# hyrise/hyrise

Measured on AMD Instinct MI355X. Metric: rows/sec TableScan+JoinHash, TPC-H SF10 lineitem, higher is better.
Workload: dtype u16

## Files before the change

hyrise_amd/csrc/join.hip:

```cpp
#include "hy_device.hpp"
#include "hy_decode.hpp"
#include "hy_arithmetic.hpp"
#include "hy_scan_job.hpp"

#include <algorithm>
#include <atomic>
#include <cmath>
#include <chrono>
#include <cstring>
#include <type_traits>

namespace hy {

constexpr uint32_t JOIN_TILE = 4096;
constexpr uint32_t JOIN_THREADS = 512;
constexpr uint32_t JOIN_WAVES = JOIN_THREADS / 64;
constexpr uint32_t JOIN_WAVE_ROWS = JOIN_TILE / JOIN_WAVES;
constexpr uint32_t JOIN_ROUNDS = JOIN_WAVE_ROWS / 64;
constexpr uint32_t JOIN_STAGE = JOIN_TILE + 256;
constexpr uint32_t MAX_PARTITIONS = 256;
typedef uint32_t u32x2_t __attribute__((ext_vector_type(2)));
typedef uint32_t u32x4_t __attribute__((ext_vector_type(4)));
constexpr uint32_t PROBE_SIZE_PER_CHUNK = 65535u * 2u;
constexpr uint32_t BLOOM_BITS = 1u << 20;
// ... 2140 lines not shown
  hipLaunchKernelGGL(scan_blocks, dim3(n_blocks), dim3(256), 0, stream, in, n, sums.as<uint64_t>(), out);
  return HY_OK;
}


struct JoinMailbox {
  uint64_t key_or, first_key, last_key;
  uint64_t key_min, key_max;
  uint32_t unsorted, any_null, equal_neighbours, duplicate;
  uint32_t unsorted_signed, build_unconfirmed;
  uint64_t n_pairs;
  uint32_t n_slices, n_uncached, fits;
  uint32_t error;
};
static thread_local JoinMailbox* t_mailbox = nullptr;
static thread_local JoinMailbox* t_mailbox_dev = nullptr;

struct BuildVerdict {
  uint64_t key_min, key_max;
  uint32_t unsorted_signed, equal_neighbours, outside_hint, done;
};

struct ZeroedBlocks {
  void* table = nullptr;
  size_t table_capacity = 0;
  void* filter = nullptr;
  size_t dirty_table = 0, dirty_filter = 0;
  bool clean = false;
  hipStream_t stream = nullptr;
};
static thread_local ZeroedBlocks t_zeroed[2];

static void free_zeroed_blocks() {
  for (ZeroedBlocks& z : t_zeroed) {
    if (z.table) (void)hipFree(z.table);
    if (z.filter) (void)hipFree(z.filter);
    z = ZeroedBlocks{};
  }
}

void release_thread_join_state() {
  if (t_mailbox) (void)hipHostFree(t_mailbox);
  t_mailbox = t_mailbox_dev = nullptr;
  free_zeroed_blocks();
}

static hy_status join_mailbox(JoinMailbox** host, JoinMailbox** device) {
  if (!t_mailbox) {
    static_assert(sizeof(JoinMailbox) <= 256, "the mailbox is a 256-byte pinned block");
    HY_HIP(hipHostMalloc(reinterpret_cast<void**>(&t_mailbox), 256, hipHostMallocMapped));
    HY_HIP(hipHostGetDevicePointer(reinterpret_cast<void**>(&t_mailbox_dev), t_mailbox, 0));
  }
  std::memset(t_mailbox, 0, sizeof(JoinMailbox));
  *host = t_mailbox;
  *device = t_mailbox_dev;
  return HY_OK;
}

// ... 216 lines not shown
    low = other_low < low ? other_low : low;
    high = other_high > high ? other_high : high;
  }
  __syncthreads();
  if ((tid & 63) == 0) { s_min[tid >> 6] = low; s_max[tid >> 6] = high; atomicOr(&s_flags, static_cast<uint32_t>(bits)); }
  __syncthreads();
  if (tid != 0) return;
  for (uint32_t w = 0; w < 4; ++w) { low = s_min[w] < low ? s_min[w] : low; high = s_max[w] > high ? s_max[w] : high; }
  verdict->key_min = low ^ SIGN;
  verdict->key_max = high ^ SIGN;
  verdict->unsorted_signed = s_flags & 1u ? 1 : 0;
  verdict->equal_neighbours = s_flags & 2u ? 1 : 0;
  verdict->outside_hint = s_flags & 4u ? 1 : 0;
  verdict->done = 1;
  __threadfence_system();
}

constexpr uint32_t FW_STEP = 512;
constexpr uint32_t FW_STEPS_PER_SLICE = SLICE_ROWS / FW_STEP;
constexpr uint32_t FW_WINDOW = 2048;
static_assert(HY_FOR_BLOCK_SIZE % FW_STEP == 0, "a step lies in one FrameOfReference block");

constexpr uint32_t FW_BATCH = 4;

struct FillWaveState {
  uint64_t unsorted = 0, equal = 0, outside = 0;
  int32_t low = 0x7FFFFFFF, high = static_cast<int32_t>(0x80000000u);
  bool any_rows = false;
  int32_t carry = 0;
  bool has_carry = false;
};

template <uint32_t WIDTH>
__device__ __forceinline__ int32_t fill_step_key(const u32x4_t& a, const u32x4_t& b, uint32_t bias, uint32_t j) {
  uint32_t stored;
  if constexpr (WIDTH == 4) stored = j < 4 ? a[j] : b[j - 4];
  else if constexpr (WIDTH == 2) stored = (a[j / 2] >> (16 * (j & 1))) & 0xFFFFu;
  else stored = (a[j / 4] >> (8 * (j & 3))) & 0xFFu;
  return static_cast<int32_t>(stored + bias);
}

__device__ __forceinline__ bool key_in_front_of_step(const MaterializeArgs& a, uint32_t step, int32_t* key) {
  uint32_t slice = step / FW_STEPS_PER_SLICE;
  const uint32_t offset = (step % FW_STEPS_PER_SLICE) * FW_STEP;
  if (offset > 0) {
    const SliceView view = a.views[slice];
    if (view.row_count > 0) { *key = view_key(view, view.row_begin + (offset <= view.row_count ? offset : view.row_count) - 1); return true; }
  }
  while (slice-- > 0) {
    const SliceView earlier = a.views[slice];
    if (earlier.row_count == 0) continue;
    *key = view_key(earlier, earlier.row_begin + earlier.row_count - 1);
    return true;
  }
  return false;
}

__device__ __forceinline__ void fill_flush_window(const uint32_t* bits_window, uint32_t span, uint32_t first_word, uint32_t origin_word, uint32_t first_rank, bool first_is_leader, uint32_t lane,
                                                  u32x2_entry_t* entries, uint32_t* bloom_words, uint32_t debug) {
  uint32_t keys_before = 0;
  for (uint32_t begin = 0; begin < span; begin += 64) {
    const uint32_t i = begin + lane;
    const uint32_t bits = i < span ? bits_window[i] : 0u;
    const uint32_t count = __popc(bits);
    uint32_t inclusive = count;
#pragma unroll
    for (int d = 1; d < 64; d <<= 1) {
      const uint32_t other = __shfl_up(inclusive, d, 64);
      if (lane >= static_cast<uint32_t>(d)) inclusive += other;
    }
    const uint32_t base = first_rank + keys_before + inclusive - count;
    keys_before += __builtin_amdgcn_readlane(inclusive, 63);
    if (i >= span) continue;
    const uint32_t table_word = first_word + i;
    if (bits && bloom_words) atomicOr(bloom_words + ((table_word + origin_word) & (BLOOM_BITS / 32 - 1)), bits);
#ifdef HY_DEBUG_SWITCHES
    if (debug & 2) { if (bits == 0xDEADBEEFu && base == 0x12345678u) entries[0] = u32x2_entry_t{bits, base}; continue; }
#endif
    if (i == 0 || i + 1 == span) {
      if (bits) atomicOr(reinterpret_cast<uint32_t*>(entries + table_word), bits);
      if (bits && (i != 0 || first_is_leader)) reinterpret_cast<uint32_t*>(entries + table_word)[1] = base;
    } else {
      entries[table_word] = u32x2_entry_t{bits, bits ? base : 0u};
    }
  }
}

template <uint32_t WIDTH, uint32_t K>
__device__ __forceinline__ bool fill_process_steps(FillWaveState& w, const u32x4_t (&a)[K], const u32x4_t (&b)[K], const uint32_t (&bias)[K], const uint32_t (&rows)[K],
                                                   const uint32_t (&first_rank)[K], uint32_t lane, uint32_t origin, uint32_t range, u32x2_entry_t* entries, uint32_t* bloom_words,
                                                   uint32_t* bits_window, uint32_t debug) {
  const uint32_t origin_word = origin >> 5;
  if (rows[0] == 0) return true;
  int32_t key[K][8];
  uint32_t lane_rows[K];
  int32_t first_key = 0, last_key = 0;
#pragma unroll
  for (uint32_t k = 0; k < K; ++k) {
#pragma unroll
    for (uint32_t j = 0; j < 8; ++j) key[k][j] = fill_step_key<WIDTH>(a[k], b[k], bias[k], j);
    lane_rows[k] = lane * 8 < rows[k] ? (rows[k] - lane * 8 < 8 ? rows[k] - lane * 8 : 8) : 0;
    if (rows[k] != 0) {
      const uint32_t last_lane = (rows[k] - 1) >> 3, last_j = (rows[k] - 1) & 7;
      int32_t mine = key[k][0];
#pragma unroll
      for (uint32_t j = 1; j < 8; ++j) mine = last_j == j ? key[k][j] : mine;
      last_key = __builtin_amdgcn_readlane(mine, last_lane);
    }
    if (k == 0) first_key = __builtin_amdgcn_readfirstlane(key[0][0]);
  }
  const uint32_t first_rel = static_cast<uint32_t>(first_key) - origin, last_rel = static_cast<uint32_t>(last_key) - origin;
  const uint32_t first_word = first_rel >> 5;
  const bool windowed = first_rel <= range && last_rel <= range && last_rel >= first_rel && (last_rel >> 5) - first_word < FW_WINDOW;
  if (K > 1 && !windowed) return false;
  const uint32_t span = windowed ? (last_rel >> 5) - first_word + 1 : 0;
  if (!w.any_rows) w.low = first_key;
  w.high = last_key;
  w.any_rows = true;
  int32_t before[K];
  bool first_has_before[K];
  {
    int32_t carry = w.carry;
    bool has_carry = w.has_carry;
#pragma unroll
    for (uint32_t k = 0; k < K; ++k) {
      before[k] = __shfl_up(key[k][7], 1, 64);
      if (lane == 0) before[k] = carry;
      first_has_before[k] = lane != 0 || has_carry;
#pragma unroll
      for (uint32_t j = 0; j < 8; ++j) {
        const int32_t previous = j == 0 ? before[k] : key[k][j - 1];
        const bool checked = j < lane_rows[k] && (j != 0 || first_has_before[k]);
        w.unsorted |= __ballot(checked && key[k][j] < previous);
        w.equal |= __ballot(checked && key[k][j] == previous);
      }
      if (rows[k] != 0) {
        carry = __builtin_amdgcn_readlane(key[k][7], 63);
        has_carry = true;
      }
    }
  }
  const uint32_t carry_rel = static_cast<uint32_t>(w.carry) - origin;
  const bool first_is_leader = !w.has_carry || carry_rel > range || (carry_rel >> 5) != first_word;
  w.carry = last_key;
  w.has_carry = true;
  if (first_rel > range || last_rel > range) w.outside = 1;
#ifdef HY_DEBUG_SWITCHES
  if (debug & 8) return true;
#endif
  if (windowed) {
#ifdef HY_DEBUG_SWITCHES
    if (debug & 4) return true;
#endif
    for (uint32_t i = lane; i < span; i += 64) bits_window[i] = 0;
    __builtin_amdgcn_fence(__ATOMIC_RELEASE, "wavefront");
    __builtin_amdgcn_wave_barrier();
#pragma unroll
    for (uint32_t k = 0; k < K; ++k) {
#pragma unroll
      for (uint32_t j = 0; j < 8; ++j) {
        const uint32_t rel = static_cast<uint32_t>(key[k][j]) - origin;
        const uint32_t at = (rel >> 5) - first_word;
        if (j < lane_rows[k] && at < span) atomicOr(&bits_window[at], 1u << (rel & 31));
      }
    }
    __builtin_amdgcn_fence(__ATOMIC_RELEASE, "wavefront");
    __builtin_amdgcn_wave_barrier();
    __builtin_amdgcn_fence(__ATOMIC_ACQUIRE, "wavefront");
    fill_flush_window(bits_window, span, first_word, origin_word, first_rank[0], first_is_leader, lane, entries, bloom_words, debug);
    __builtin_amdgcn_wave_barrier();
  } else {
#pragma unroll
    for (uint32_t k = 0; k < K; ++k) {
      const uint32_t lane_rank = first_rank[k] + lane * 8;
#pragma unroll
      for (uint32_t j = 0; j < 8; ++j) {
        const uint32_t rel = static_cast<uint32_t>(key[k][j]) - origin;
        const int32_t previous = j == 0 ? before[k] : key[k][j - 1];
        const bool has_previous = j != 0 || first_has_before[k];
        w.outside |= __ballot(j < lane_rows[k] && rel > range);
        if (j < lane_rows[k] && rel <= range) {
          const uint32_t table_word = rel >> 5, bits = 1u << (rel & 31);
          atomicOr(reinterpret_cast<uint32_t*>(entries + table_word), bits);
          const uint32_t previous_rel = static_cast<uint32_t>(previous) - origin;
          if (!has_previous || previous_rel > range || (previous_rel >> 5) != table_word) reinterpret_cast<uint32_t*>(entries + table_word)[1] = lane_rank + j;
          if (bloom_words) atomicOr(bloom_words + ((table_word + origin_word) & (BLOOM_BITS / 32 - 1)), bits);
        }
      }
    }
  }
  return true;
}

template <uint32_t WIDTH>
struct FillBatch {
  u32x4_t a[FW_BATCH], b[FW_BATCH];
  uint32_t bias[FW_BATCH], rows[FW_BATCH], first_rank[FW_BATCH];
};

template <uint32_t WIDTH>
__device__ __forceinline__ void load_fill_batch(const MaterializeArgs& a, uint32_t batch_step, uint32_t end_step, uint32_t chunk_rows, uint32_t lane, FillBatch<WIDTH>& batch) {
  typedef const __attribute__((address_space(1))) u32x4_t* global_x4;
  typedef const __attribute__((address_space(1))) u32x2_t* global_x2;
  const uint32_t slice0 = batch_step / FW_STEPS_PER_SLICE;
  const SliceView view0 = a.views[slice0];
  const SliceView view1 = a.views[slice0 + 1 < a.n_slices ? slice0 + 1 : slice0];
  const uint32_t rank0 = view0.chunk * chunk_rows + view0.row_begin, rank1 = view1.chunk * chunk_rows + view1.row_begin;
#pragma unroll
  for (uint32_t k = 0; k < FW_BATCH; ++k) {
    const uint32_t step = batch_step + k;
    const bool second = step / FW_STEPS_PER_SLICE != slice0;
    const SliceView& view = second ? view1 : view0;
    const uint32_t offset = (step % FW_STEPS_PER_SLICE) * FW_STEP;
    batch.rows[k] = step < end_step && view.row_count > offset ? (view.row_count - offset < FW_STEP ? view.row_count - offset : FW_STEP) : 0;
    batch.first_rank[k] = (second ? rank1 : rank0) + offset;
    batch.a[k] = u32x4_t{0, 0, 0, 0};
    batch.b[k] = u32x4_t{0, 0, 0, 0};
    batch.bias[k] = 0;
    if (batch.rows[k] != 0) {
      const uint32_t row = view.row_begin + offset + (lane * 8 < batch.rows[k] ? lane * 8 : 0);
      const char* base = static_cast<const char*>(view.data);
      if constexpr (WIDTH == 4) {
        batch.a[k] = *(global_x4)(base + size_t{row} * 4);
        batch.b[k] = *(global_x4)(base + size_t{row} * 4 + 16);
      } else if constexpr (WIDTH == 2) {
        batch.a[k] = *(global_x4)(base + size_t{row} * 2);
      } else {
        const u32x2_t v = *(global_x2)(base + row);
        batch.a[k].x = v.x;
        batch.a[k].y = v.y;
      }
      if (view.kind != VIEW_INT32) batch.bias[k] = static_cast<uint32_t>(static_cast<const int32_t*>(view.aux)[(view.row_begin + offset) / HY_FOR_BLOCK_SIZE]);
    }
  }
}

struct FillCleaning {
  u32x4_t* first;
  u32x4_t* second;
  uint32_t first_vectors, second_vectors;
};

template <uint32_t WIDTH>
__global__ __launch_bounds__(256, 4) void rank_table_fill_waves(MaterializeArgs a, uint64_t key_min, uint64_t hint_range, u32x2_entry_t* entries, uint64_t* partials, uint32_t chunk_rows,
                                                             uint32_t batches_per_wave, uint32_t n_steps, uint32_t debug) {
  __shared__ uint32_t s_window[4][FW_WINDOW];
  __shared__ uint64_t s_min[4], s_max[4];
  __shared__ uint32_t s_flags;
  const uint32_t tid = threadIdx.x, lane = tid & 63, wave = __builtin_amdgcn_readfirstlane(tid >> 6);
  constexpr uint64_t SIGN = 1ull << 63;
  const uint32_t origin = static_cast<uint32_t>(key_min), range = static_cast<uint32_t>(hint_range);
  uint32_t* bloom_words = reinterpret_cast<uint32_t*>(a.bloom_out);
  uint32_t* bits_window = s_window[wave];
  const uint32_t steps_per_wave = batches_per_wave * FW_BATCH;
  const uint32_t first_step = (blockIdx.x * 4 + wave) * steps_per_wave;
  const uint32_t end_step = first_step + steps_per_wave < n_steps ? first_step + steps_per_wave : n_steps;
  if (tid == 0) s_flags = 0;
  FillWaveState w;
  FillBatch<WIDTH> current, ahead;
  if (first_step < end_step) {
    load_fill_batch<WIDTH>(a, first_step, end_step, chunk_rows, lane, current);
    int32_t front = 0;
    uint32_t has_front = 0;
    if (lane == 0) has_front = key_in_front_of_step(a, first_step, &front) ? 1u : 0u;
    w.carry = __builtin_amdgcn_readfirstlane(front);
    w.has_carry = __builtin_amdgcn_readfirstlane(has_front) != 0;
  }
  for (uint32_t batch_step = first_step; batch_step < end_step; batch_step += FW_BATCH) {
    if (batch_step + FW_BATCH < end_step) load_fill_batch<WIDTH>(a, batch_step + FW_BATCH, end_step, chunk_rows, lane, ahead);
    bool packed = true;
#pragma unroll
    for (uint32_t k = 1; k < FW_BATCH; ++k) packed = packed && (current.rows[k] == 0 || current.rows[k - 1] == FW_STEP);
    if (!packed || !fill_process_steps<WIDTH, FW_BATCH>(w, current.a, current.b, current.bias, current.rows, current.first_rank, lane, origin, range, entries, bloom_words, bits_window,
                                                        debug)) {
#pragma unroll
      for (uint32_t k = 0; k < FW_BATCH; ++k) {
        const u32x4_t one_a[1] = {current.a[k]}, one_b[1] = {current.b[k]};
        const uint32_t one_bias[1] = {current.bias[k]}, one_rows[1] = {current.rows[k]}, one_rank[1] = {current.first_rank[k]};
        fill_process_steps<WIDTH, 1>(w, one_a, one_b, one_bias, one_rows, one_rank, lane, origin, range, entries, bloom_words, bits_window, debug);
      }
    }
    current = ahead;
  }
  const uint64_t unsorted = w.unsorted, equal = w.equal, outside = w.outside;
  const int32_t low = w.low, high = w.high;
  const bool any_rows = w.any_rows;
  const uint32_t flags = (unsorted ? 1u : 0u) | (equal ? 2u : 0u) | (outside ? 4u : 0u);
  if (lane == 0) {
    s_min[wave] = any_rows ? static_cast<uint64_t>(static_cast<int64_t>(low)) ^ SIGN : ~0ull;
    s_max[wave] = any_rows ? static_cast<uint64_t>(static_cast<int64_t>(high)) ^ SIGN : 0;
  }
  __syncthreads();
  if (lane == 0 && flags) atomicOr(&s_flags, flags);
  __syncthreads();
  if (tid == 0) {
    uint64_t group_low = ~0ull, group_high = 0;
    for (uint32_t v = 0; v < 4; ++v) { group_low = s_min[v] < group_low ? s_min[v] : group_low; group_high = s_max[v] > group_high ? s_max[v] : group_high; }
    uint64_t* record = partials + 4 * size_t{blockIdx.x};
    record[0] = group_low;
    record[1] = group_high;
    record[2] = s_flags;
  }
}

template <typename K>
__global__ void publish_build_flags(const uint32_t* flags, const K* keys, uint64_t n, JoinMailbox* mailbox) {
// ... 112 lines not shown

__global__ void publish_join_status(hy_join_status* status, uint64_t n_pairs, uint32_t n_slices, uint32_t fits) {
  status->n_pairs = n_pairs;
  status->n_slices = n_slices;
  status->fits = fits;
  status->build_confirmed = 1;
  status->error = 0;
  status->reserved = 0;
}

struct StageClock {
  bool on = HY_DEBUG_ENV("HY_JOIN_TIMING") != nullptr;
  std::chrono::steady_clock::time_point start = std::chrono::steady_clock::now();
  void mark(const char* what) {
    if (on) fprintf(stderr, "  join %-28s %8.1f us\n", what, std::chrono::duration<double, std::micro>(std::chrono::steady_clock::now() - start).count());
  }
};

static uint32_t device_cu_count();
static bool lds_atomics_are_lane_ordered(hipStream_t stream);

struct BuildSide {
  DeviceBuffer keys, rows, keys_tmp, rows_tmp, dir, bloom, flags, rank_entries, partials;
  FillCleaning cleaning{nullptr, nullptr, 0, 0};
  ZeroedBlocks* cleaned = nullptr;
  bool hint_allows_duplicates = false;
  bool bloom_is_bits = false;
  bool hinted = false;
  uint64_t hint_min = 0, hint_max = 0;
  const BuildVerdict* verdict = nullptr;
  const uint64_t* fill_records = nullptr;
  uint32_t n_fill_records = 0;
  uint64_t n = 0;
  Directory directory{};
  RankTable rank{};
  bool any_null = false;
};

template <bool KEY32, bool ID32>
struct BuildTypes {
  static constexpr bool key32 = KEY32, id32 = ID32;
  using Key = typename BuildKey<KEY32>::type;
  using Row = typename BuildRow<ID32>::type;
};
template <typename F>
static auto with_build_types(bool key32, bool id32, F&& f) {
  if (key32 && id32) return f(BuildTypes<true, true>{});
// ... 88 lines not shown
  BuildPlan plan;
  BuildSide& b;
  hipStream_t stream;
  MaterializeArgs m{};
  DeviceBuffer counts, offsets;
  uint64_t total = 0;
};

static void identity_table(BuildJob& job, u32x2_t* entries, uint64_t key_min, uint64_t key_max) {
  BuildSide& b = job.b;
  b.rank.entries = entries;
  b.rank.key_min = key_min;
  b.rank.range = key_max - key_min;
  b.rank.identity_rows = job.column->host_segments[0].size;
  b.rank.identity_inverse = 1.0 / static_cast<double>(b.rank.identity_rows);
  Directory& d = b.directory;
  d = Directory{};
  d.n = job.total;
  d.key_min = key_min;
  d.key_max = key_max;
  d.n_buckets = 1;
}

static hy_status take_zeroed_block(BuildJob& job, size_t table_vectors, size_t bloom_vectors, bool* taken) {
  BuildSide& b = job.b;
  hipStream_t stream = job.stream;
  *taken = false;
  if (!FIXED_JOIN_CLEAN_TABLES || table_vectors + bloom_vectors >= (1ull << 31)) return HY_OK;
  if ((t_zeroed[0].table && t_zeroed[0].stream != stream) || (t_zeroed[1].table && t_zeroed[1].stream != stream)) {
    HY_HIP(hipDeviceSynchronize());
    free_zeroed_blocks();
  }
  int mine = -1;
  for (int i = 0; i < 2; ++i) if (t_zeroed[i].clean && t_zeroed[i].table_capacity >= 16 * table_vectors) mine = i;
  if (mine < 0) {
    mine = !t_zeroed[0].table ? 0 : !t_zeroed[1].table ? 1 : t_zeroed[1].clean && !t_zeroed[0].clean ? 1 : 0;
    ZeroedBlocks& z = t_zeroed[mine];
    if (z.table_capacity < 16 * table_vectors) {
      if (z.table) { HY_HIP(hipStreamSynchronize(stream)); HY_HIP(hipFree(z.table)); z.table = nullptr; }
      z.table_capacity = (16 * table_vectors * 5 / 4 + 4095) & ~size_t{4095};
      HY_HIP(hipMalloc(&z.table, z.table_capacity));
      if (!z.filter) HY_HIP(hipMalloc(&z.filter, BLOOM_BITS / 8));
      z.stream = stream;
      z.clean = false;
      z.dirty_table = z.table_capacity;
      z.dirty_filter = BLOOM_BITS / 8;
    }
  }
  ZeroedBlocks& z = t_zeroed[mine];
  ZeroedBlocks& other = t_zeroed[1 - mine];
  if (!z.clean) {
    hipLaunchKernelGGL(zero_vectors, dim3(static_cast<uint32_t>(std::min<size_t>(2048, (z.dirty_table / 16 + z.dirty_filter / 16 + 255) / 256))), dim3(256), 0, stream,
                       static_cast<u32x4_t*>(z.table), z.dirty_table / 16, static_cast<u32x4_t*>(z.filter), z.dirty_filter / 16);
  }
  if (other.table && !other.clean) {
    b.cleaning = FillCleaning{static_cast<u32x4_t*>(other.table), static_cast<u32x4_t*>(other.filter), static_cast<uint32_t>(other.dirty_table / 16), static_cast<uint32_t>(other.dirty_filter / 16)};
    b.cleaned = &other;
  }
  z.clean = false;
  z.dirty_table = 16 * table_vectors;
  z.dirty_filter = 16 * bloom_vectors;
  b.rank_entries.borrow(z.table);
  if (job.wants.bloom) { b.bloom.borrow(z.filter); job.m.bloom_out = b.bloom.as<uint8_t>(); }
  *taken = true;
  return HY_OK;
}

static void block_cleaning_queued(BuildSide& b) {
  if (b.cleaned) { b.cleaned->clean = true; b.cleaned->dirty_table = b.cleaned->dirty_filter = 0; }
}

static hy_status launch_hinted_fill(BuildJob& job, uint32_t stream_width, uint64_t origin, uint64_t hint_range, u32x2_t* entries, uint32_t* tickets, BuildVerdict* verdict) {
  BuildSide& b = job.b;
  MaterializeArgs m = job.m;
  const uint32_t n_slices = job.column->n_slices;
  uint32_t fill_debug = 0;
  if (const char* debug = HY_DEBUG_ENV("HY_JOIN_FILL_DEBUG")) {
    fill_debug = static_cast<uint32_t>(atoi(debug));
    if (fill_debug & 1) m.bloom_out = nullptr;
    if (atoi(debug) >= 2 && !option(HY_OPT_JOIN_FILL_WGS_PER_CU)) m.keep_nulls = 0xFFFFFFFFu;
  }
  hipEvent_t fill_started = nullptr, fill_stopped = nullptr;
  profile_events(&fill_started, &fill_stopped, HY_KERNEL_JOIN_BUILD);
  if (!stream_width) {
    hipExtLaunchKernelGGL(rank_table_fill_checked, dim3(n_slices), dim3(256), 0, job.stream, fill_started, fill_stopped, 0, m, origin, hint_range, entries, b.partials.as<uint64_t>(), tickets, verdict);
    b.verdict = verdict;
    return HY_OK;
  }
  auto with_width = [&](auto f) { return stream_width == 4 ? f(std::integral_constant<uint32_t, 4>{}) : stream_width == 2 ? f(std::integral_constant<uint32_t, 2>{}) : f(std::integral_constant<uint32_t, 1>{}); };
  int per_cu = 0;
  HY_TRY(with_width([&](auto w) -> hy_status {
    HY_HIP(hipOccupancyMaxActiveBlocksPerMultiprocessor(&per_cu, reinterpret_cast<const void*>(rank_table_fill_waves<decltype(w)::value>), 256, 0));
    return HY_OK;
  }));
  const uint32_t fill_waves = 4 * device_cu_count() * static_cast<uint32_t>(std::max<int64_t>(1, std::min<int64_t>(per_cu, option(HY_OPT_JOIN_FILL_WGS_PER_CU))));
  const uint32_t n_steps = n_slices * FW_STEPS_PER_SLICE, n_batches = (n_steps + FW_BATCH - 1) / FW_BATCH;
  const uint32_t batches_per_wave = (n_batches + fill_waves - 1) / fill_waves, waves = (n_batches + batches_per_wave - 1) / batches_per_wave, groups = (waves + 3) / 4;
  b.fill_records = b.partials.as<uint64_t>();
  b.n_fill_records = groups;
  with_width([&](auto w) {
    hipExtLaunchKernelGGL(rank_table_fill_waves<decltype(w)::value>, dim3(groups), dim3(256), 0, job.stream, fill_started, fill_stopped, 0, m, origin, hint_range, entries, b.partials.as<uint64_t>(),
                          job.column->host_segments[0].size, batches_per_wave, n_steps, fill_debug);
    return HY_OK;
  });
  return HY_OK;
}

static hy_status fill_hinted(BuildJob& job) {
  BuildSide& b = job.b;
  const hy_column* build = job.column;
  const uint64_t key_min = build->join_hint.key_min.load(std::memory_order_relaxed);
  uint64_t key_max = build->join_hint.key_max.load(std::memory_order_relaxed);
  if (option(HY_OPT_JOIN_BREAK_HINT) && key_max - key_min > 64) key_max -= 64;
  const uint64_t origin = key_min & ~uint64_t{31};
  const uint64_t words = ((key_max - origin) >> 5) + 1;
  const size_t ticket_bytes = 128 * (size_t{CHECKED_FILL_TICKETS} + 1);
  const size_t table_bytes = 8 * (words + 2) + ticket_bytes + 64;
  const size_t table_vectors = (table_bytes + 15) / 16, bloom_vectors = job.wants.bloom ? BLOOM_BITS / 8 / 16 : 0;
  uint32_t stream_width = build->stream_width == 1 || build->stream_width == 2 || build->stream_width == 4 ? build->stream_width : 0;
  if (option(HY_OPT_JOIN_FILL_WGS_PER_CU) <= 0) stream_width = 0;
  HY_TRY(b.partials.alloc(32 * (size_t{build->n_slices} * FW_STEPS_PER_SLICE / 4 + 1)));
  bool zeroed = false;
  if (stream_width) HY_TRY(take_zeroed_block(job, table_vectors, bloom_vectors, &zeroed));
  if (!zeroed) {
    HY_TRY(b.rank_entries.alloc(table_bytes));
    hipLaunchKernelGGL(zero_vectors, dim3(static_cast<uint32_t>(std::min<size_t>(2048, (table_vectors + bloom_vectors + 255) / 256))), dim3(256), 0, job.stream,
                       b.rank_entries.as<u32x4_t>(), table_vectors, b.bloom.as<u32x4_t>(), bloom_vectors);
  }
  u32x2_t* entries = b.rank_entries.as<u32x2_t>();
  uint32_t* tickets = reinterpret_cast<uint32_t*>(entries + words + 2);
  HY_TRY(launch_hinted_fill(job, stream_width, origin, key_max - origin, entries, tickets, reinterpret_cast<BuildVerdict*>(reinterpret_cast<char*>(tickets) + ticket_bytes)));
  identity_table(job, entries, origin, key_max);
  b.directory.key_min = key_min;
  b.bloom_is_bits = job.wants.bloom;
  b.hinted = true;
  b.hint_allows_duplicates = job.wants.existence_only;
  b.hint_min = key_min;
  b.hint_max = key_max;
  return HY_OK;
}

static hy_status fill_identity(BuildJob& job, bool* built) {
  BuildSide& b = job.b;
  const hy_column* build = job.column;
  const uint32_t n_slices = build->n_slices;
  *built = false;
  uint32_t first_slice = n_slices, last_slice = 0, slice = 0;
  for (uint32_t c = 0; c < build->n_chunks; ++c) {
    const uint32_t size = build->host_segments[c].size;
    const uint32_t chunk_slices = std::max<uint32_t>(1, (size + SLICE_ROWS - 1) / SLICE_ROWS);
// ... 1149 lines not shown
```

hyrise_amd/csrc/join_pkfk.hpp:

```cpp
#pragma once

#ifndef HY_PK_TILE
#define HY_PK_TILE 8192
#endif
#ifndef HY_PK_WAVES_PER_SIMD
#define HY_PK_WAVES_PER_SIMD 4
#endif
constexpr uint32_t PK_TILE = HY_PK_TILE;
constexpr uint32_t PK_TILES_PER_SLICE = SLICE_ROWS / PK_TILE;
constexpr uint32_t PK_ROUNDS = 16;
constexpr uint32_t PK_THREADS = PK_TILE / PK_ROUNDS;
constexpr uint32_t PK_WAVES = PK_THREADS / 64;
constexpr uint32_t PK_WAVE_ROWS = PK_TILE / PK_WAVES;
constexpr uint32_t PK_COUNT_WAVE_ROWS = 2048;
constexpr uint32_t PK_COUNT_THREADS = 64 * (PK_TILE / PK_COUNT_WAVE_ROWS);
constexpr uint32_t PK_COUNT_BATCHES = PK_COUNT_WAVE_ROWS / 512;
constexpr uint32_t PK_SCAN_THREADS = 512;
constexpr uint32_t PK_SCAN_CHUNK = 8192;
static_assert(SLICE_ROWS % PK_TILE == 0 && HY_FOR_BLOCK_SIZE % PK_WAVE_ROWS == 0 && HY_FOR_BLOCK_SIZE == PK_COUNT_WAVE_ROWS && PK_TILE % PK_COUNT_WAVE_ROWS == 0,
              "a wave's rows must lie in one FrameOfReference block");
static_assert(PK_TILE <= (1u << 13), "a staged pair keeps its row in 13 bits");

struct PkArgs {
  const SliceView* views;
// ... 814 lines not shown
  for (uint32_t i = 0; i < wave * PK_ROUNDS; ++i) { members_before += s_members[i]; emitters_before += s_emitters[i]; }
  const uint64_t lower_lanes = (1ull << lane) - 1;
  const uint64_t cell_base = a.origin_pairs[partition] + a.rel_pairs[static_cast<size_t>(partition) * a.stride + tile];
#pragma unroll
  for (uint32_t k = 0; k < PK_ROUNDS; ++k) {
    const bool member = (members[k] >> lane) & 1;
    if (member && members_before + __popcll(members[k] & lower_lanes) == cut_rank) a.slice_offsets[slice] = cell_base + emitters_before + __popcll(emitters[k] & lower_lanes);
    members_before += __popcll(members[k]);
    emitters_before += __popcll(emitters[k]);
  }
}

__global__ __launch_bounds__(PK_THREADS) void pk_cuts(PkArgs a) {
  __shared__ __attribute__((aligned(16))) uint32_t s_cut[PK_WAVES * 1024 + 2 * PK_WAVES * PK_ROUNDS];
  const uint32_t tid = threadIdx.x;
  pk_cut_slice(a, blockIdx.x, s_cut, tid, tid & 63, __builtin_amdgcn_readfirstlane(tid >> 6));
}

template <bool INNER, bool MASKS = false, bool RANKS = false>
__global__ __launch_bounds__(PK_THREADS, HY_PK_WAVES_PER_SIMD) void pk_emit(PkArgs a) {
  extern __shared__ __attribute__((aligned(16))) uint32_t join_smem[];
  const uint32_t partitions = 1u << a.radix_bits;
  const uint32_t tid = threadIdx.x, lane = tid & 63, wave = __builtin_amdgcn_readfirstlane(tid >> 6);
  for (uint32_t i = blockIdx.x * PK_THREADS + tid; i < a.cleaning.first_vectors + a.cleaning.second_vectors; i += gridDim.x * PK_THREADS) {
    if (i < a.cleaning.first_vectors) a.cleaning.first[i] = u32x4_t{0, 0, 0, 0}; else a.cleaning.second[i - a.cleaning.first_vectors] = u32x4_t{0, 0, 0, 0};
  }
  if (blockIdx.x < a.cut_blocks) { pk_cut_slice<MASKS>(a, blockIdx.x, join_smem, tid, lane, wave); return; }
  const uint32_t block = blockIdx.x - a.cut_blocks;
  uint32_t tile;
  if (a.emit_group_shift < 32) {
    const uint32_t xcd = block & 7, j = block >> 3, shift = a.emit_group_shift;
    const uint32_t whole = ((a.n_tiles + 7) / 8) >> shift << shift;
    tile = j < whole ? ((j >> shift) << (shift + 3)) + (xcd << shift) + (j & ((1u << shift) - 1)) : whole * 8 + (j - whole) * 8 + xcd;
  } else tile = (block & 7) * ((a.n_tiles + 7) / 8) + (block >> 3);
  if (tile >= a.n_tiles) return;
  const SliceView view = pk_tile_view(a, tile);
  const uint32_t fits = a.plan->fits;
  if (!fits || view.row_count == 0) return;
  const size_t cell = static_cast<size_t>(tid < partitions ? tid : 0) * a.stride + tile;
  const uint32_t cell_pairs = tid < partitions ? a.counts[cell] >> 16 : 0;
  const uint32_t cell_base = static_cast<uint32_t>(a.origin_pairs[tid < partitions ? tid : 0]) + a.rel_pairs[cell];
  pk_emit_tile<INNER, MASKS, RANKS>(a, tile, view, cell_pairs, cell_base, join_smem, tid, lane, wave);
}
```

Baseline: 366.0 billion.

## Write every rank-table word during the streamed fill instead of pre-zeroing the table

The streamed build fill now walks the key range in order and writes each table word itself, storing explicit zeros for empty stretches and carrying a pending partial word between batches. This removes the separate zeroing pass and the pooled pre-zeroed table blocks; only the bloom filter keeps the cached zeroed-block scheme. To keep that valid, sparse key ranges and ranges near the 32-bit limit fall back to the zeroed path, and a closing step finishes the tail of each wave's span. The price is more complex ordering logic across waves, plus a gap-closing look-ahead that can write extra zeros.

```diff
diff --git a/hyrise_amd/csrc/join.hip b/hyrise_amd/csrc/join.hip
--- a/hyrise_amd/csrc/join.hip
+++ b/hyrise_amd/csrc/join.hip
@@ -2186,10 +2186,7 @@
 };
 
 struct ZeroedBlocks {
-  void* table = nullptr;
-  size_t table_capacity = 0;
   void* filter = nullptr;
-  size_t dirty_table = 0, dirty_filter = 0;
   bool clean = false;
   hipStream_t stream = nullptr;
 };
@@ -2197,7 +2194,6 @@
 
 static void free_zeroed_blocks() {
   for (ZeroedBlocks& z : t_zeroed) {
-    if (z.table) (void)hipFree(z.table);
     if (z.filter) (void)hipFree(z.filter);
     z = ZeroedBlocks{};
   }
@@ -2460,6 +2456,9 @@
 static_assert(HY_FOR_BLOCK_SIZE % FW_STEP == 0, "a step lies in one FrameOfReference block");
 
 constexpr uint32_t FW_BATCH = 4;
+constexpr uint64_t FW_SPARSE_WORDS_PER_KEY = 2;
+constexpr uint64_t FW_RANGE_LIMIT = (uint64_t{1} << 32) - uint64_t{FW_WINDOW} * 32;
+static_assert(FW_STEPS_PER_SLICE % FW_BATCH == 0 && FW_WINDOW % 2 == 0, "a batch lies in one slice; the window leaves in pairs of words");
 
 struct FillWaveState {
   uint64_t unsorted = 0, equal = 0, outside = 0;
@@ -2467,6 +2466,9 @@
   bool any_rows = false;
   int32_t carry = 0;
   bool has_carry = false;
+  bool started = false;
+  uint32_t cursor = 0;
+  uint32_t pending_bits = 0, pending_base = 0;
 };
 
 template <uint32_t WIDTH>
@@ -2494,146 +2496,10 @@
   return false;
 }
 
-__device__ __forceinline__ void fill_flush_window(const uint32_t* bits_window, uint32_t span, uint32_t first_word, uint32_t origin_word, uint32_t first_rank, bool first_is_leader, uint32_t lane,
-                                                  u32x2_entry_t* entries, uint32_t* bloom_words, uint32_t debug) {
-  uint32_t keys_before = 0;
-  for (uint32_t begin = 0; begin < span; begin += 64) {
-    const uint32_t i = begin + lane;
-    const uint32_t bits = i < span ? bits_window[i] : 0u;
-    const uint32_t count = __popc(bits);
-    uint32_t inclusive = count;
-#pragma unroll
-    for (int d = 1; d < 64; d <<= 1) {
-      const uint32_t other = __shfl_up(inclusive, d, 64);
-      if (lane >= static_cast<uint32_t>(d)) inclusive += other;
-    }
-    const uint32_t base = first_rank + keys_before + inclusive - count;
-    keys_before += __builtin_amdgcn_readlane(inclusive, 63);
-    if (i >= span) continue;
-    const uint32_t table_word = first_word + i;
-    if (bits && bloom_words) atomicOr(bloom_words + ((table_word + origin_word) & (BLOOM_BITS / 32 - 1)), bits);
-#ifdef HY_DEBUG_SWITCHES
-    if (debug & 2) { if (bits == 0xDEADBEEFu && base == 0x12345678u) entries[0] = u32x2_entry_t{bits, base}; continue; }
-#endif
-    if (i == 0 || i + 1 == span) {
-      if (bits) atomicOr(reinterpret_cast<uint32_t*>(entries + table_word), bits);
-      if (bits && (i != 0 || first_is_leader)) reinterpret_cast<uint32_t*>(entries + table_word)[1] = base;
-    } else {
-      entries[table_word] = u32x2_entry_t{bits, bits ? base : 0u};
-    }
-  }
-}
-
-template <uint32_t WIDTH, uint32_t K>
-__device__ __forceinline__ bool fill_process_steps(FillWaveState& w, const u32x4_t (&a)[K], const u32x4_t (&b)[K], const uint32_t (&bias)[K], const uint32_t (&rows)[K],
-                                                   const uint32_t (&first_rank)[K], uint32_t lane, uint32_t origin, uint32_t range, u32x2_entry_t* entries, uint32_t* bloom_words,
-                                                   uint32_t* bits_window, uint32_t debug) {
-  const uint32_t origin_word = origin >> 5;
-  if (rows[0] == 0) return true;
-  int32_t key[K][8];
-  uint32_t lane_rows[K];
-  int32_t first_key = 0, last_key = 0;
-#pragma unroll
-  for (uint32_t k = 0; k < K; ++k) {
-#pragma unroll
-    for (uint32_t j = 0; j < 8; ++j) key[k][j] = fill_step_key<WIDTH>(a[k], b[k], bias[k], j);
-    lane_rows[k] = lane * 8 < rows[k] ? (rows[k] - lane * 8 < 8 ? rows[k] - lane * 8 : 8) : 0;
-    if (rows[k] != 0) {
-      const uint32_t last_lane = (rows[k] - 1) >> 3, last_j = (rows[k] - 1) & 7;
-      int32_t mine = key[k][0];
-#pragma unroll
-      for (uint32_t j = 1; j < 8; ++j) mine = last_j == j ? key[k][j] : mine;
-      last_key = __builtin_amdgcn_readlane(mine, last_lane);
-    }
-    if (k == 0) first_key = __builtin_amdgcn_readfirstlane(key[0][0]);
-  }
-  const uint32_t first_rel = static_cast<uint32_t>(first_key) - origin, last_rel = static_cast<uint32_t>(last_key) - origin;
-  const uint32_t first_word = first_rel >> 5;
-  const bool windowed = first_rel <= range && last_rel <= range && last_rel >= first_rel && (last_rel >> 5) - first_word < FW_WINDOW;
-  if (K > 1 && !windowed) return false;
-  const uint32_t span = windowed ? (last_rel >> 5) - first_word + 1 : 0;
-  if (!w.any_rows) w.low = first_key;
-  w.high = last_key;
-  w.any_rows = true;
-  int32_t before[K];
-  bool first_has_before[K];
-  {
-    int32_t carry = w.carry;
-    bool has_carry = w.has_carry;
-#pragma unroll
-    for (uint32_t k = 0; k < K; ++k) {
-      before[k] = __shfl_up(key[k][7], 1, 64);
-      if (lane == 0) before[k] = carry;
-      first_has_before[k] = lane != 0 || has_carry;
-#pragma unroll
-      for (uint32_t j = 0; j < 8; ++j) {
-        const int32_t previous = j == 0 ? before[k] : key[k][j - 1];
-        const bool checked = j < lane_rows[k] && (j != 0 || first_has_before[k]);
-        w.unsorted |= __ballot(checked && key[k][j] < previous);
-        w.equal |= __ballot(checked && key[k][j] == previous);
-      }
-      if (rows[k] != 0) {
-        carry = __builtin_amdgcn_readlane(key[k][7], 63);
-        has_carry = true;
-      }
-    }
-  }
-  const uint32_t carry_rel = static_cast<uint32_t>(w.carry) - origin;
-  const bool first_is_leader = !w.has_carry || carry_rel > range || (carry_rel >> 5) != first_word;
-  w.carry = last_key;
-  w.has_carry = true;
-  if (first_rel > range || last_rel > range) w.outside = 1;
-#ifdef HY_DEBUG_SWITCHES
-  if (debug & 8) return true;
-#endif
-  if (windowed) {
-#ifdef HY_DEBUG_SWITCHES
-    if (debug & 4) return true;
-#endif
-    for (uint32_t i = lane; i < span; i += 64) bits_window[i] = 0;
-    __builtin_amdgcn_fence(__ATOMIC_RELEASE, "wavefront");
-    __builtin_amdgcn_wave_barrier();
-#pragma unroll
-    for (uint32_t k = 0; k < K; ++k) {
-#pragma unroll
-      for (uint32_t j = 0; j < 8; ++j) {
-        const uint32_t rel = static_cast<uint32_t>(key[k][j]) - origin;
-        const uint32_t at = (rel >> 5) - first_word;
-        if (j < lane_rows[k] && at < span) atomicOr(&bits_window[at], 1u << (rel & 31));
-      }
-    }
-    __builtin_amdgcn_fence(__ATOMIC_RELEASE, "wavefront");
-    __builtin_amdgcn_wave_barrier();
-    __builtin_amdgcn_fence(__ATOMIC_ACQUIRE, "wavefront");
-    fill_flush_window(bits_window, span, first_word, origin_word, first_rank[0], first_is_leader, lane, entries, bloom_words, debug);
-    __builtin_amdgcn_wave_barrier();
-  } else {
-#pragma unroll
-    for (uint32_t k = 0; k < K; ++k) {
-      const uint32_t lane_rank = first_rank[k] + lane * 8;
-#pragma unroll
-      for (uint32_t j = 0; j < 8; ++j) {
-        const uint32_t rel = static_cast<uint32_t>(key[k][j]) - origin;
-        const int32_t previous = j == 0 ? before[k] : key[k][j - 1];
-        const bool has_previous = j != 0 || first_has_before[k];
-        w.outside |= __ballot(j < lane_rows[k] && rel > range);
-        if (j < lane_rows[k] && rel <= range) {
-          const uint32_t table_word = rel >> 5, bits = 1u << (rel & 31);
-          atomicOr(reinterpret_cast<uint32_t*>(entries + table_word), bits);
-          const uint32_t previous_rel = static_cast<uint32_t>(previous) - origin;
-          if (!has_previous || previous_rel > range || (previous_rel >> 5) != table_word) reinterpret_cast<uint32_t*>(entries + table_word)[1] = lane_rank + j;
-          if (bloom_words) atomicOr(bloom_words + ((table_word + origin_word) & (BLOOM_BITS / 32 - 1)), bits);
-        }
-      }
-    }
-  }
-  return true;
-}
-
 template <uint32_t WIDTH>
 struct FillBatch {
   u32x4_t a[FW_BATCH], b[FW_BATCH];
-  uint32_t bias[FW_BATCH], rows[FW_BATCH], first_rank[FW_BATCH];
+  uint32_t bias[FW_BATCH], rows[FW_BATCH], first_rank;
 };
 
 template <uint32_t WIDTH>
@@ -2651,7 +2517,7 @@
     const SliceView& view = second ? view1 : view0;
     const uint32_t offset = (step % FW_STEPS_PER_SLICE) * FW_STEP;
     batch.rows[k] = step < end_step && view.row_count > offset ? (view.row_count - offset < FW_STEP ? view.row_count - offset : FW_STEP) : 0;
-    batch.first_rank[k] = (second ? rank1 : rank0) + offset;
+    if (k == 0) batch.first_rank = (second ? rank1 : rank0) + offset;
     batch.a[k] = u32x4_t{0, 0, 0, 0};
     batch.b[k] = u32x4_t{0, 0, 0, 0};
     batch.bias[k] = 0;
@@ -2673,16 +2539,232 @@
   }
 }
 
+__device__ __forceinline__ void fill_store_zeros(u32x2_entry_t* entries, uint32_t lo, uint32_t hi, uint32_t lane) {
+  if (lo >= hi) return;
+  if (lo & 1) {
+    if (lane == 0) entries[lo] = u32x2_entry_t{0, 0};
+    ++lo;
+  }
+  const uint32_t pairs = (hi - lo) >> 1;
+  u32x4_t* vectors = reinterpret_cast<u32x4_t*>(entries + lo);
+  for (uint32_t i = lane; i < pairs; i += 64) vectors[i] = u32x4_t{0, 0, 0, 0};
+  if (((hi - lo) & 1) && lane == 0) entries[hi - 1] = u32x2_entry_t{0, 0};
+}
+
+__device__ __forceinline__ void fill_store_word(u32x2_entry_t* entries, uint32_t* bloom_words, uint32_t table_word, uint32_t origin_word, uint32_t bits, uint32_t base, uint32_t lane) {
+  if (lane != 0) return;
+  entries[table_word] = u32x2_entry_t{bits, bits ? base : 0u};
+  if (bits && bloom_words) atomicOr(bloom_words + ((table_word + origin_word) & (BLOOM_BITS / 32 - 1)), bits);
+}
+
+__device__ __forceinline__ void fill_flush_piece(const uint32_t* bits_window, uint32_t span, uint32_t piece, uint32_t lo, uint32_t hi, uint32_t need, uint32_t* keys_before, uint32_t first_rank,
+                                                 uint32_t pending_bits, uint32_t pending_base, uint32_t origin_word, uint32_t lane, u32x2_entry_t* entries, uint32_t* bloom_words, uint32_t debug) {
+#ifdef HY_DEBUG_SWITCHES
+  const bool wide = !(debug & 2);
+#else
+  constexpr bool wide = true;
+#endif
+  for (uint32_t begin = 0; begin < span; begin += 128) {
+    const uint32_t i = begin + 2 * lane;
+    const u32x2_t own = i < span ? *reinterpret_cast<const u32x2_t*>(bits_window + i) : u32x2_t{0, 0};
+    const uint32_t count0 = __popc(own.x), count = count0 + __popc(own.y);
+    uint32_t inclusive = count;
+#pragma unroll
+    for (int d = 1; d < 64; d <<= 1) {
+      const uint32_t other = __shfl_up(inclusive, d, 64);
+      if (lane >= static_cast<uint32_t>(d)) inclusive += other;
+    }
+    const uint32_t before = *keys_before + inclusive - count;
+    *keys_before += __builtin_amdgcn_readlane(inclusive, 63);
+    const uint32_t word0 = piece + i, word1 = word0 + 1;
+    uint32_t bits0 = own.x, base0 = first_rank + before, bits1 = own.y, base1 = first_rank + before + count0;
+    if (pending_bits && word0 == lo) { bits0 |= pending_bits; base0 = pending_base; }
+    if (pending_bits && word1 == lo) { bits1 |= pending_bits; base1 = pending_base; }
+    const bool mine0 = word0 >= lo && word0 < hi && before + count0 >= need, mine1 = word1 >= lo && word1 < hi && before + count >= need;
+    if (wide && mine0 && mine1) *reinterpret_cast<u32x4_t*>(entries + word0) = u32x4_t{bits0, bits0 ? base0 : 0u, bits1, bits1 ? base1 : 0u};
+    else {
+      if (mine0) entries[word0] = u32x2_entry_t{bits0, bits0 ? base0 : 0u};
+      if (mine1) entries[word1] = u32x2_entry_t{bits1, bits1 ? base1 : 0u};
+    }
+    if (bloom_words) {
+      const uint32_t fold0 = mine0 ? bits0 : 0u, fold1 = mine1 ? bits1 : 0u;
+#pragma unroll
+      for (uint32_t half = 0; half < 2; ++half) {
+        const uint32_t holder = half * 32 + (lane >> 1);
+        const uint32_t even = __shfl(fold0, holder, 64), odd = __shfl(fold1, holder, 64);
+        const uint32_t folded = lane & 1 ? odd : even;
+        if (folded) atomicOr(bloom_words + ((piece + begin + half * 64 + lane + origin_word) & (BLOOM_BITS / 32 - 1)), folded);
+      }
+    }
+  }
+}
+
+template <uint32_t WIDTH>
+__device__ __forceinline__ void fill_process_batch(FillWaveState& w, const FillBatch<WIDTH>& batch, uint32_t lane, uint32_t origin, uint32_t range, u32x2_entry_t* entries,
+                                                   uint32_t* bloom_words, uint32_t* bits_window, uint32_t debug) {
+  constexpr uint32_t K = FW_BATCH;
+  const uint32_t origin_word = origin >> 5;
+  const uint32_t (&rows)[K] = batch.rows;
+  if (rows[0] == 0) return;
+  int32_t key[K][8];
+  uint32_t lane_rows[K];
+  int32_t first_key = 0, last_key = 0;
+  uint32_t total = 0;
+#pragma unroll
+  for (uint32_t k = 0; k < K; ++k) {
+#pragma unroll
+    for (uint32_t j = 0; j < 8; ++j) key[k][j] = fill_step_key<WIDTH>(batch.a[k], batch.b[k], batch.bias[k], j);
+    lane_rows[k] = lane * 8 < rows[k] ? (rows[k] - lane * 8 < 8 ? rows[k] - lane * 8 : 8) : 0;
+    total += rows[k];
+    if (rows[k] != 0) {
+      const uint32_t last_lane = (rows[k] - 1) >> 3, last_j = (rows[k] - 1) & 7;
+      int32_t mine = key[k][0];
+#pragma unroll
+      for (uint32_t j = 1; j < 8; ++j) mine = last_j == j ? key[k][j] : mine;
+      last_key = __builtin_amdgcn_readlane(mine, last_lane);
+    }
+    if (k == 0) first_key = __builtin_amdgcn_readfirstlane(key[0][0]);
+  }
+  const uint32_t first_rel = static_cast<uint32_t>(first_key) - origin, last_rel = static_cast<uint32_t>(last_key) - origin;
+  if (!w.any_rows) w.low = first_key;
+  w.high = last_key;
+  w.any_rows = true;
+  {
+    int32_t carry = w.carry;
+    bool has_carry = w.has_carry;
+#pragma unroll
+    for (uint32_t k = 0; k < K; ++k) {
+      int32_t before = __shfl_up(key[k][7], 1, 64);
+      if (lane == 0) before = carry;
+      const bool first_has_before = lane != 0 || has_carry;
+#pragma unroll
+      for (uint32_t j = 0; j < 8; ++j) {
+        const int32_t previous = j == 0 ? before : key[k][j - 1];
+        const bool checked = j < lane_rows[k] && (j != 0 || first_has_before);
+        w.unsorted |= __ballot(checked && key[k][j] < previous);
+        w.equal |= __ballot(checked && key[k][j] == previous);
+      }
+      if (rows[k] != 0) {
+        carry = __builtin_amdgcn_readlane(key[k][7], 63);
+        has_carry = true;
+      }
+    }
+  }
+  w.carry = last_key;
+  w.has_carry = true;
+  if (first_rel > range || last_rel > range) w.outside = 1;
+  if (w.unsorted | w.outside) return;
+#ifdef HY_DEBUG_SWITCHES
+  if (debug & 12) return;
+#endif
+  const uint32_t first_word = first_rel >> 5, last_word = last_rel >> 5;
+  if (w.started && w.pending_bits && first_word > w.cursor) {
+    fill_store_word(entries, bloom_words, w.cursor, origin_word, w.pending_bits, w.pending_base, lane);
+    w.pending_bits = 0;
+    ++w.cursor;
+  }
+  const uint32_t front_word = w.cursor - 1;
+  uint32_t keys_before = 0, need = w.started ? 0u : 1u;
+  uint32_t piece = (w.started ? w.cursor : front_word) & ~1u;
+  for (bool first_piece = true;; first_piece = false, piece += FW_WINDOW) {
+    const uint32_t span = last_word - piece < FW_WINDOW ? last_word - piece + 1 : FW_WINDOW;
+    const uint32_t piece_key = origin + (piece << 5);
+    bool holds = false;
+#pragma unroll
+    for (uint32_t k = 0; k < K; ++k) {
+      const uint32_t lowest = (static_cast<uint32_t>(key[k][0]) - origin) >> 5, highest = (static_cast<uint32_t>(key[k][7]) - origin) >> 5;
+      holds = holds || (lane_rows[k] != 0 && lowest < piece + span && (lane_rows[k] < 8 || highest >= piece));
+    }
+    if (__ballot(holds)) {
+      for (uint32_t i = lane; i < ((span + 1) & ~1u); i += 64) bits_window[i] = 0;
+      __builtin_amdgcn_fence(__ATOMIC_RELEASE, "wavefront");
+      __builtin_amdgcn_wave_barrier();
+#pragma unroll
+      for (uint32_t k = 0; k < K; ++k) {
+#pragma unroll
+        for (uint32_t j = 0; j < 8; ++j) {
+          const uint32_t rel = static_cast<uint32_t>(key[k][j]) - piece_key;
+          const uint32_t at = rel >> 5;
+          if (j < lane_rows[k] && at < span) atomicOr(&bits_window[at], 1u << (rel & 31));
+        }
+      }
+      __builtin_amdgcn_fence(__ATOMIC_RELEASE, "wavefront");
+      __builtin_amdgcn_wave_barrier();
+      __builtin_amdgcn_fence(__ATOMIC_ACQUIRE, "wavefront");
+      if (!w.started && first_piece) need = __popc(bits_window[front_word - piece]) + 1;
+      fill_flush_piece(bits_window, span, piece, w.cursor, last_word, need, &keys_before, batch.first_rank, w.pending_bits, w.pending_base, origin_word, lane, entries, bloom_words, debug);
+      if (last_word - piece < FW_WINDOW) break;
+      __builtin_amdgcn_wave_barrier();
+    } else if (keys_before >= need) {
+      fill_store_zeros(entries, piece > w.cursor ? piece : w.cursor, piece + span, lane);
+    }
+  }
+  const uint32_t last_bits = __builtin_amdgcn_readfirstlane(bits_window[last_word - piece]);
+  __builtin_amdgcn_wave_barrier();
+  if (!w.started && last_word == front_word) return;
+  if (!(w.pending_bits && last_word == w.cursor)) {
+    w.pending_bits = 0;
+    w.pending_base = batch.first_rank + total - __popc(last_bits);
+  }
+  w.pending_bits |= last_bits;
+  w.started = true;
+  w.cursor = last_word;
+}
+
+constexpr uint32_t FW_MAX_AHEAD = 4096;
+__device__ __forceinline__ void fill_close_span(const MaterializeArgs& a, FillWaveState& w, uint32_t end_step, uint32_t max_ahead, uint32_t lane, uint32_t origin, uint32_t range,
+                                                u32x2_entry_t* entries, uint32_t* bloom_words) {
+  if (!w.any_rows || !w.started || (w.unsorted | w.outside)) return;
+  const uint32_t table_end = (range >> 5) + 1;
+  uint32_t slice = end_step / FW_STEPS_PER_SLICE, offset = (end_step % FW_STEPS_PER_SLICE) * FW_STEP;
+  uint32_t bits = 0, next = w.cursor + 1;
+  bool closed = false;
+  for (uint32_t seen = 0; !closed && seen < max_ahead;) {
+    const uint32_t want = max_ahead - seen < 64 ? max_ahead - seen : 64;
+    int32_t key = 0;
+    bool have = false;
+    uint32_t got = 0;
+    while (got < want && slice < a.n_slices) {
+      const SliceView view = a.views[slice];
+      const uint32_t rows = view.row_count > offset ? view.row_count - offset : 0, take = rows < want - got ? rows : want - got;
+      if (lane >= got && lane < got + take) {
+        key = view_key(view, view.row_begin + offset + (lane - got));
+        have = true;
+      }
+      got += take;
+      offset += take;
+      if (offset >= view.row_count) { ++slice; offset = 0; }
+    }
+    const uint32_t rel = static_cast<uint32_t>(key) - origin, table_word = rel >> 5;
+    const bool inside = have && rel <= range;
+    bits |= inside && table_word == w.cursor ? 1u << (rel & 31) : 0u;
+    const uint64_t later = __ballot(inside && table_word > w.cursor);
+    if (later) {
+      next = __shfl(table_word, __ffsll(static_cast<long long>(later)) - 1, 64);
+      closed = true;
+    } else if (got < want) {
+      next = table_end;
+      closed = true;
+    }
+    seen += got;
+  }
+  if (!closed) w.outside = 1;
+#pragma unroll
+  for (int d = 32; d > 0; d >>= 1) bits |= __shfl_xor(bits, d, 64);
+  next = next < table_end ? next : table_end;
+  fill_store_word(entries, bloom_words, w.cursor, origin >> 5, w.pending_bits | bits, w.pending_base, lane);
+  fill_store_zeros(entries, w.cursor + 1, next, lane);
+}
+
 struct FillCleaning {
-  u32x4_t* first;
-  u32x4_t* second;
-  uint32_t first_vectors, second_vectors;
+  u32x4_t* filter;
+  uint32_t vectors;
 };
 
 template <uint32_t WIDTH>
 __global__ __launch_bounds__(256, 4) void rank_table_fill_waves(MaterializeArgs a, uint64_t key_min, uint64_t hint_range, u32x2_entry_t* entries, uint64_t* partials, uint32_t chunk_rows,
-                                                             uint32_t batches_per_wave, uint32_t n_steps, uint32_t debug) {
-  __shared__ uint32_t s_window[4][FW_WINDOW];
+                                                             uint32_t batches_per_wave, uint32_t n_steps, uint32_t max_ahead, uint32_t debug) {
+  __shared__ __attribute__((aligned(16))) uint32_t s_window[4][FW_WINDOW];
   __shared__ uint64_t s_min[4], s_max[4];
   __shared__ uint32_t s_flags;
   const uint32_t tid = threadIdx.x, lane = tid & 63, wave = __builtin_amdgcn_readfirstlane(tid >> 6);
@@ -2703,23 +2785,17 @@
     if (lane == 0) has_front = key_in_front_of_step(a, first_step, &front) ? 1u : 0u;
     w.carry = __builtin_amdgcn_readfirstlane(front);
     w.has_carry = __builtin_amdgcn_readfirstlane(has_front) != 0;
+    const uint32_t front_rel = static_cast<uint32_t>(w.carry) - origin;
+    w.started = !w.has_carry;
+    if (w.has_carry && front_rel > range) w.outside = 1;
+    w.cursor = w.has_carry ? (front_rel >> 5) + 1 : 0;
   }
   for (uint32_t batch_step = first_step; batch_step < end_step; batch_step += FW_BATCH) {
     if (batch_step + FW_BATCH < end_step) load_fill_batch<WIDTH>(a, batch_step + FW_BATCH, end_step, chunk_rows, lane, ahead);
-    bool packed = true;
-#pragma unroll
-    for (uint32_t k = 1; k < FW_BATCH; ++k) packed = packed && (current.rows[k] == 0 || current.rows[k - 1] == FW_STEP);
-    if (!packed || !fill_process_steps<WIDTH, FW_BATCH>(w, current.a, current.b, current.bias, current.rows, current.first_rank, lane, origin, range, entries, bloom_words, bits_window,
-                                                        debug)) {
-#pragma unroll
-      for (uint32_t k = 0; k < FW_BATCH; ++k) {
-        const u32x4_t one_a[1] = {current.a[k]}, one_b[1] = {current.b[k]};
-        const uint32_t one_bias[1] = {current.bias[k]}, one_rows[1] = {current.rows[k]}, one_rank[1] = {current.first_rank[k]};
-        fill_process_steps<WIDTH, 1>(w, one_a, one_b, one_bias, one_rows, one_rank, lane, origin, range, entries, bloom_words, bits_window, debug);
-      }
-    }
+    fill_process_batch<WIDTH>(w, current, lane, origin, range, entries, bloom_words, bits_window, debug);
     current = ahead;
   }
+  fill_close_span(a, w, end_step, max_ahead, lane, origin, range, entries, bloom_words);
   const uint64_t unsorted = w.unsorted, equal = w.equal, outside = w.outside;
   const int32_t low = w.low, high = w.high;
   const bool any_rows = w.any_rows;
@@ -2878,7 +2954,7 @@
 
 struct BuildSide {
   DeviceBuffer keys, rows, keys_tmp, rows_tmp, dir, bloom, flags, rank_entries, partials;
-  FillCleaning cleaning{nullptr, nullptr, 0, 0};
+  FillCleaning cleaning{nullptr, 0};
   ZeroedBlocks* cleaned = nullptr;
   bool hint_allows_duplicates = false;
   bool bloom_is_bits = false;
@@ -3013,52 +3089,39 @@
   d.n_buckets = 1;
 }
 
-static hy_status take_zeroed_block(BuildJob& job, size_t table_vectors, size_t bloom_vectors, bool* taken) {
+static hy_status take_zeroed_block(BuildJob& job, bool* taken) {
   BuildSide& b = job.b;
   hipStream_t stream = job.stream;
+  constexpr size_t filter_vectors = BLOOM_BITS / 8 / 16;
   *taken = false;
-  if (!FIXED_JOIN_CLEAN_TABLES || table_vectors + bloom_vectors >= (1ull << 31)) return HY_OK;
-  if ((t_zeroed[0].table && t_zeroed[0].stream != stream) || (t_zeroed[1].table && t_zeroed[1].stream != stream)) {
+  if (!FIXED_JOIN_CLEAN_TABLES) return HY_OK;
+  if ((t_zeroed[0].filter && t_zeroed[0].stream != stream) || (t_zeroed[1].filter && t_zeroed[1].stream != stream)) {
     HY_HIP(hipDeviceSynchronize());
     free_zeroed_blocks();
   }
-  int mine = -1;
-  for (int i = 0; i < 2; ++i) if (t_zeroed[i].clean && t_zeroed[i].table_capacity >= 16 * table_vectors) mine = i;
+  int mine = t_zeroed[0].clean ? 0 : t_zeroed[1].clean ? 1 : -1;
   if (mine < 0) {
-    mine = !t_zeroed[0].table ? 0 : !t_zeroed[1].table ? 1 : t_zeroed[1].clean && !t_zeroed[0].clean ? 1 : 0;
+    mine = !t_zeroed[0].filter ? 0 : !t_zeroed[1].filter ? 1 : 0;
     ZeroedBlocks& z = t_zeroed[mine];
-    if (z.table_capacity < 16 * table_vectors) {
-      if (z.table) { HY_HIP(hipStreamSynchronize(stream)); HY_HIP(hipFree(z.table)); z.table = nullptr; }
-      z.table_capacity = (16 * table_vectors * 5 / 4 + 4095) & ~size_t{4095};
-      HY_HIP(hipMalloc(&z.table, z.table_capacity));
-      if (!z.filter) HY_HIP(hipMalloc(&z.filter, BLOOM_BITS / 8));
-      z.stream = stream;
-      z.clean = false;
-      z.dirty_table = z.table_capacity;
-      z.dirty_filter = BLOOM_BITS / 8;
-    }
+    if (!z.filter) HY_HIP(hipMalloc(&z.filter, 16 * filter_vectors));
+    z.stream = stream;
+    hipLaunchKernelGGL(zero_vectors, dim3(static_cast<uint32_t>((filter_vectors + 255) / 256)), dim3(256), 0, stream, static_cast<u32x4_t*>(z.filter), filter_vectors, static_cast<u32x4_t*>(nullptr), size_t{0});
   }
   ZeroedBlocks& z = t_zeroed[mine];
   ZeroedBlocks& other = t_zeroed[1 - mine];
-  if (!z.clean) {
-    hipLaunchKernelGGL(zero_vectors, dim3(static_cast<uint32_t>(std::min<size_t>(2048, (z.dirty_table / 16 + z.dirty_filter / 16 + 255) / 256))), dim3(256), 0, stream,
-                       static_cast<u32x4_t*>(z.table), z.dirty_table / 16, static_cast<u32x4_t*>(z.filter), z.dirty_filter / 16);
-  }
-  if (other.table && !other.clean) {
-    b.cleaning = FillCleaning{static_cast<u32x4_t*>(other.table), static_cast<u32x4_t*>(other.filter), static_cast<uint32_t>(other.dirty_table / 16), static_cast<uint32_t>(other.dirty_filter / 16)};
+  if (other.filter && !other.clean) {
+    b.cleaning = FillCleaning{static_cast<u32x4_t*>(other.filter), static_cast<uint32_t>(filter_vectors)};
     b.cleaned = &other;
   }
   z.clean = false;
-  z.dirty_table = 16 * table_vectors;
-  z.dirty_filter = 16 * bloom_vectors;
-  b.rank_entries.borrow(z.table);
-  if (job.wants.bloom) { b.bloom.borrow(z.filter); job.m.bloom_out = b.bloom.as<uint8_t>(); }
+  b.bloom.borrow(z.filter);
+  job.m.bloom_out = b.bloom.as<uint8_t>();
   *taken = true;
   return HY_OK;
 }
 
 static void block_cleaning_queued(BuildSide& b) {
-  if (b.cleaned) { b.cleaned->clean = true; b.cleaned->dirty_table = b.cleaned->dirty_filter = 0; }
+  if (b.cleaned) b.cleaned->clean = true;
 }
 
 static hy_status launch_hinted_fill(BuildJob& job, uint32_t stream_width, uint64_t origin, uint64_t hint_range, u32x2_t* entries, uint32_t* tickets, BuildVerdict* verdict) {
@@ -3091,7 +3154,7 @@
   b.n_fill_records = groups;
   with_width([&](auto w) {
     hipExtLaunchKernelGGL(rank_table_fill_waves<decltype(w)::value>, dim3(groups), dim3(256), 0, job.stream, fill_started, fill_stopped, 0, m, origin, hint_range, entries, b.partials.as<uint64_t>(),
-                          job.column->host_segments[0].size, batches_per_wave, n_steps, fill_debug);
+                          job.column->host_segments[0].size, batches_per_wave, n_steps, job.wants.existence_only ? FW_MAX_AHEAD : 32u, fill_debug);
     return HY_OK;
   });
   return HY_OK;
@@ -3110,13 +3173,15 @@
   const size_t table_vectors = (table_bytes + 15) / 16, bloom_vectors = job.wants.bloom ? BLOOM_BITS / 8 / 16 : 0;
   uint32_t stream_width = build->stream_width == 1 || build->stream_width == 2 || build->stream_width == 4 ? build->stream_width : 0;
   if (option(HY_OPT_JOIN_FILL_WGS_PER_CU) <= 0) stream_width = 0;
+  if (words > FW_SPARSE_WORDS_PER_KEY * job.total) stream_width = 0;
+  if (key_max - origin >= FW_RANGE_LIMIT) stream_width = 0;
   HY_TRY(b.partials.alloc(32 * (size_t{build->n_slices} * FW_STEPS_PER_SLICE / 4 + 1)));
+  HY_TRY(b.rank_entries.alloc(table_bytes));
   bool zeroed = false;
-  if (stream_width) HY_TRY(take_zeroed_block(job, table_vectors, bloom_vectors, &zeroed));
-  if (!zeroed) {
-    HY_TRY(b.rank_entries.alloc(table_bytes));
-    hipLaunchKernelGGL(zero_vectors, dim3(static_cast<uint32_t>(std::min<size_t>(2048, (table_vectors + bloom_vectors + 255) / 256))), dim3(256), 0, job.stream,
-                       b.rank_entries.as<u32x4_t>(), table_vectors, b.bloom.as<u32x4_t>(), bloom_vectors);
+  if (stream_width && job.wants.bloom) HY_TRY(take_zeroed_block(job, &zeroed));
+  if (!stream_width || (job.wants.bloom && !zeroed)) {
+    hipLaunchKernelGGL(zero_vectors, dim3(static_cast<uint32_t>(std::min<size_t>(2048, ((stream_width ? 0 : table_vectors) + bloom_vectors + 255) / 256))), dim3(256), 0, job.stream,
+                       b.rank_entries.as<u32x4_t>(), stream_width ? size_t{0} : table_vectors, b.bloom.as<u32x4_t>(), bloom_vectors);
   }
   u32x2_t* entries = b.rank_entries.as<u32x2_t>();
   uint32_t* tickets = reinterpret_cast<uint32_t*>(entries + words + 2);
diff --git a/hyrise_amd/csrc/join_pkfk.hpp b/hyrise_amd/csrc/join_pkfk.hpp
--- a/hyrise_amd/csrc/join_pkfk.hpp
+++ b/hyrise_amd/csrc/join_pkfk.hpp
@@ -860,9 +860,7 @@
   extern __shared__ __attribute__((aligned(16))) uint32_t join_smem[];
   const uint32_t partitions = 1u << a.radix_bits;
   const uint32_t tid = threadIdx.x, lane = tid & 63, wave = __builtin_amdgcn_readfirstlane(tid >> 6);
-  for (uint32_t i = blockIdx.x * PK_THREADS + tid; i < a.cleaning.first_vectors + a.cleaning.second_vectors; i += gridDim.x * PK_THREADS) {
-    if (i < a.cleaning.first_vectors) a.cleaning.first[i] = u32x4_t{0, 0, 0, 0}; else a.cleaning.second[i - a.cleaning.first_vectors] = u32x4_t{0, 0, 0, 0};
-  }
+  for (uint32_t i = blockIdx.x * PK_THREADS + tid; i < a.cleaning.vectors; i += gridDim.x * PK_THREADS) a.cleaning.filter[i] = u32x4_t{0, 0, 0, 0};
   if (blockIdx.x < a.cut_blocks) { pk_cut_slice<MASKS>(a, blockIdx.x, join_smem, tid, lane, wave); return; }
   const uint32_t block = blockIdx.x - a.cut_blocks;
   uint32_t tile;
```

After: 372.0 billion (median of 6 runs). 1.6% higher.
